# heracles-ec/heracles

Measured on AMD Instinct MI355X. Metric: map->Cl pairs/sec + mixing-matrix build sec, nside=4096 lmax=6144, higher is better.
Workload: dtype f64

## Files before the change

### heracles_amd/_lib.py

```python

from __future__ import annotations

import ctypes as C
import os
import threading

import numpy as np

_HERE = os.path.dirname(os.path.abspath(__file__))
_LIBNAME = os.environ.get("HX_LIBRARY") or os.path.join(_HERE, "libhxsht.so")
_lock = threading.Lock()
_lib = None

HX_OK = 0
HX_ERR_ARG, HX_ERR_NO_DEVICE, HX_ERR_HIP, HX_ERR_MEM, HX_ERR_UNSUPPORTED = -1, -2, -3, -4, -5

SYMBOLS = (
    "hx_version", "hx_last_error", "hx_device_count", "hx_init", "hx_set_stream",
    "hx_get_stream", "hx_set_async", "hx_synchronize", "hx_timer_start", "hx_timer_stop",
    "hx_profile_enable", "hx_profile_reset", "hx_profile_get", "hx_plan_create", "hx_set_max_lds_fft",
    "hx_plan_destroy", "hx_plan_scratch_bytes", "hx_plan_release_scratch", "hx_set_scratch_budget", "hx_plan_last_chunks", "hx_plan_mfma_flops", "hx_plan_executed_flops", "hx_executed_flops", "hx_measure_peaks", "hx_measured_mfma_clock", "hx_map2alm", "hx_map2alm_multi", "hx_map2alm_list", "hx_alm2map", "hx_copy",
    "hx_alm2cl_pairs", "hx_alm2cl_pairs_range", "hx_gauss_legendre", "hx_gauss_legendre_dd", "hx_wigner_d_table", "hx_mixmat",
    "hx_mixmat_eb", "hx_mixmat_batch", "hx_mixctx_create", "hx_mixctx_apply", "hx_mixctx_destroy", "hx_mixctx_set_bins", "hx_mixctx_apply_binned", "hx_cl2corr", "hx_corr2cl", "hx_ang2pix_ring", "hx_map_values", "hx_ud_grade", "hx_reorder", "hx_matvec", "hx_pinv", "hx_alm_resample", "hx_region_maps", "hx_alm_subtract", "hx_fits_unpack_f64", "hx_fits_pack_f64", "hx_fits_unpack_columns",
    "hx_pointsht_create", "hx_pointsht_destroy", "hx_pointsht_info", "hx_pointsht_adjoint",
    "hx_pixel_weights_size", "hx_pixel_weights_expand",
    "hx_ring_modes_size", "hx_ring_modes", "hx_legendre_from_modes", "hx_allgather_alms", "hx_host_alloc", "hx_host_free", "hx_mixmat_gemm_clock", "hx_mixmat_release", "hx_release_caches",
    "hx_cov_gram", "hx_cov_delete2", "hx_cov_shrink_sums",
    "hx_catmap_create", "hx_catmap_page", "hx_catmap_moments", "hx_catmap_finish", "hx_catmap_destroy",
    "hx_catmap_create_sel", "hx_catmap_page_sel", "hx_catmap_moments_sel", "hx_catmap_finish_sel", "hx_catmap_destroy_sel",
)


class HxError(RuntimeError):

    def __init__(self, code, msg):
        super().__init__(f"libhxsht error {code}: {msg}")
        self.code = code


def library_path() -> str:
    return _LIBNAME


def load():
# ... 5 lines not shown
            raise HxError(
                HX_ERR_NO_DEVICE,
                f"{_LIBNAME} not found: build it with `make -C heracles_amd/csrc` "
                "(hipcc, gfx950).  heracles_amd has no CPU fallback.",
            )
        try:
            import torch
        except ImportError:
            pass
        L = C.CDLL(_LIBNAME)
        vp, i, dp = C.c_void_p, C.c_int, C.c_void_p
        L.hx_version.restype = C.c_char_p
        L.hx_last_error.restype = C.c_char_p
        L.hx_get_stream.restype = vp
        L.hx_set_stream.argtypes = [vp]
        L.hx_plan_create.restype = vp
        L.hx_plan_create.argtypes = [i, i, i]
        L.hx_plan_destroy.argtypes = [vp]
        L.hx_plan_destroy.restype = None
        L.hx_plan_scratch_bytes.argtypes = [vp]
        L.hx_plan_scratch_bytes.restype = C.c_int64
        L.hx_plan_release_scratch.argtypes = [vp]
        L.hx_set_scratch_budget.argtypes = [C.c_double]
        L.hx_plan_last_chunks.argtypes = [vp]
        L.hx_plan_mfma_flops.argtypes = [vp, i, i, C.POINTER(C.c_double)]
        L.hx_plan_executed_flops.argtypes = [vp, i, i, C.POINTER(C.c_double)]
        L.hx_executed_flops.argtypes = [C.POINTER(C.c_double), i]
        L.hx_measure_peaks.argtypes = [C.POINTER(C.c_double)]
        L.hx_measured_mfma_clock.restype = C.c_double
        L.hx_map2alm.argtypes = [vp, i, i, dp, dp, dp, dp, dp, i]
        L.hx_alm2map.argtypes = [vp, i, i, dp, dp]
        L.hx_map2alm_multi.argtypes = [vp, i, vp, vp, vp, vp, dp, dp, vp]
        L.hx_map2alm_list.argtypes = [vp, i, vp, vp, vp, dp, dp, dp, dp, i]
        L.hx_copy.argtypes = [vp, vp, C.c_int64]
        L.hx_alm2cl_pairs.argtypes = [i, vp, vp, i, i, vp, vp, dp]
        L.hx_alm2cl_pairs_range.argtypes = [i, vp, vp, i, i, vp, vp, i, i, i, dp]
        L.hx_gauss_legendre.argtypes = [i, dp, dp]
        L.hx_gauss_legendre_dd.argtypes = [i, dp, dp, dp]
        L.hx_wigner_d_table.argtypes = [i, i, i, i, dp, dp]
        L.hx_mixmat.argtypes = [dp, i, i, i, i, i, i, dp]
        L.hx_mixmat_eb.argtypes = [dp, i, i, i, i, dp]
        L.hx_mixmat_batch.argtypes = [i, dp, i, i, i, i, vp, vp, vp, vp]
        L.hx_mixctx_create.restype = vp
        L.hx_mixctx_create.argtypes = [i, i, i]
        L.hx_mixctx_apply.argtypes = [vp, dp, i, i, dp]
        L.hx_mixctx_destroy.argtypes = [vp]
# ... 123 lines not shown
def release_caches():
    check(load().hx_release_caches())


def copy(dst, src):
    nb = int(src.nbytes) if hasattr(src, "nbytes") else int(src.numel() * src.element_size())
    nd = int(dst.nbytes) if hasattr(dst, "nbytes") else int(dst.numel() * dst.element_size())
    if nb != nd:
        raise ValueError(f"copy of {nb} bytes into {nd}")
    check(load().hx_copy(ptr(dst), ptr(src), nb))


def executed_flops(reset=False):
    ensure_init()
    out = (C.c_double * 2)()
    check(load().hx_executed_flops(out, 1 if reset else 0))
    return out[0], out[1]


def set_scratch_budget(nbytes: float):
    check(load().hx_set_scratch_budget(float(nbytes)))


class Timer:

    def __enter__(self):
        check(load().hx_timer_start())
        self.ms = None
        return self

    def __exit__(self, *exc):
        t = C.c_float()
        check(load().hx_timer_stop(C.byref(t)))
        self.ms = float(t.value)
        return False


def profile_enable(on=True):
    check(load().hx_profile_enable(1 if on else 0))


def profile_reset():
    check(load().hx_profile_reset())


def profile_get(name: str):
# ... 41 lines not shown
```

### heracles_amd/csrc/hx_analysis.hip

```cpp
#include <algorithm>
#include <cmath>
#include <cstdlib>
#include <cstring>

#include "hx_sht_common.h"

namespace hx {
using namespace hxfft;

constexpr int HALF_F = 1;
template <int SPIN>
struct LegCfg {
    static constexpr int NW = SPIN == 0 ? 16 : 8;
    static constexpr int NT = SPIN == 0 ? 1 : 2;
    static constexpr int NOP = SPIN == 0 ? 1 : 2;
    static constexpr int NPAR = (SPIN == 2 && HALF_F) ? 1 : 2;
};
int analysis_f_rows(int spin) { return spin == 0 ? LegCfg<0>::NPAR * LegCfg<0>::NOP : LegCfg<2>::NPAR * LegCfg<2>::NOP; }

struct LegParams {
    PlanDev P;
    const LegTask *__restrict__ tasks;
    const double *__restrict__ F;
    double *__restrict__ partial;
    int m0, ms;
    long long row0;
    int ng;
    int ncol;
    int pcol;
    const MTasks *__restrict__ of_m;
    const long long *__restrict__ arow;
    long long arow0;
    int add_all;
};

template <int SPIN>
__global__ __launch_bounds__(256) void k_fourier_combine(PlanDev P, const double2 *__restrict__ Y, int ncomp, int ng,
                                                         int ncol, int m0, int ms, const double *__restrict__ rw,
                                                         const LegTask *__restrict__ tasks, const MTasks *__restrict__ of_m,
                                                         double *__restrict__ F, int tile0)
{
    constexpr int NOP = LegCfg<SPIN>::NOP;
    __shared__ RingAtM ring_at_m[32];
    const int m = m0 + blockIdx.x * ms;
    const int ty = (int)blockIdx.y + tile0;
    const MTasks mt = of_m[m];
    if (mt.count == 0 || ty < tasks[mt.first].rb0) return;
    if (threadIdx.x < 32) ring_at_m[threadIdx.x] = ring_at_m_of(P, ty * 32 + threadIdx.x, m, rw);
    __syncthreads();
    const int rp = ty * 32 + (threadIdx.x >> 3);
    const int slot = threadIdx.x & 7;
    const bool live = rp < P.nrp;
    const RingAtM ram = ring_at_m[threadIdx.x >> 3];
    constexpr int NPAR = LegCfg<SPIN>::NPAR;
    double *row = F + (((long long)blockIdx.x * P.nrp_pad + rp) * NPAR) * NOP * ncol;
    for (int g = 0; g < ng; ++g) {
// ... 114 lines not shown
                    v[u] = make_double2(prow[j ^ 3], prow[(j + 1) ^ 3]);
                }
                if (SPIN == 2 && HALF_F && ((l + m) & 1)) {
                    if (c & 1) v[u].y = -v[u].y;
                    else v[u].x = -v[u].x;
                }
                if (alphan) al[u] = alphan[almidx(lmax, l, m)];
                if (fl) f[u] = fl[l];
            }
        }
#pragma unroll
        for (int u = 0; u < U; ++u) {
            if (!on[u]) continue;
            double2 w = v[u];
            if (alphan) { w.x *= al[u]; w.y *= al[u]; }
            if (fl) { w.x *= f[u]; w.y *= f[u]; }
            double2 *dst = alm + dsti[u];
            if (add) { const double2 o = *dst; w.x += o.x; w.y += o.y; }
            *dst = w;
        }
    }
}

template <int SPIN, int NG, int NBX, int NSUB = 1>
__global__ __launch_bounds__(256, 2) void k_legendre_duo(LegParams A, const double2 *__restrict__ coefn)
{
    using C = PipeCfg<SPIN>;
    constexpr int NW = 4, NOP = C::NOP, NCH = C::NCH, NPAIR = 16;
    constexpr int NXA = NBX > 0 ? NBX : 1;
    constexpr int DQ0 = NG * 512, DSZ = NG * 512 + NBX * 128;
    constexpr bool HALFB = SPIN == 2;
    constexpr int SB = SPIN == 2 ? DUO_SCALE_BITS2 : DUO_SCALE_BITS0;
    constexpr int GAPN = DUO_GAP >= 0 ? DUO_GAP : ((SPIN == 2 && NG == 2 && NBX == 2) ? 5 : (SPIN == 2 && NG == 2 && NBX == 1) ? 6 : (SPIN == 2 && NG == 1 && NBX == 2) ? 0 : 4);
    constexpr int GORDER = DUO_ORDER >= 0 ? DUO_ORDER : ((SPIN == 2 && NG == 2 && NBX == 2) ? 2 : (SPIN == 0 && NG == 1 && NBX == 1) ? 1 : 0);
    constexpr int NPB = HALFB ? 1 : 2;
    constexpr int TW = NSUB * DSZ > 2048 ? NSUB * DSZ : 2048;
    static_assert(NG >= 1 && NG <= 2 && TW * NW * 8 <= 81920, "two work-groups per CU");
    static_assert(SPIN == 0 || HALF_F, "spin 2: the lambda- chain carries (-1)^(l + m) lambda- (one operand row, wave-uniform coefficients)");
    __shared__ double tile[NW][TW];
    __shared__ int lead_in[2][NW];
    const PlanDev &P = A.P;
    const int m = A.m0 + blockIdx.x * A.ms, lmax = P.lmax;
    const MTasks mt = A.of_m[m];
    const int l0 = SPIN == 0 ? m : (m > 2 ? m : 2);
    const int off = (l0 + m) & 1;
    const int nblk = (lmax - l0) / LBLK + 1;
// ... 30 lines not shown
        for (int sp = 0; sp < NPAIR; ++sp) {
            const int op = SPIN == 0 ? 0 : sp & 1, q = SPIN == 0 ? sp : sp >> 1;
            const int rbq = SPIN == 0 ? 2 * w + (q >> 3) : w;
            const bool on = rbq < task.nrb;
            const long long row = (long long)blockIdx.x * P.nrp_pad + (task.rb0 + rbq) * RBLK + pipe_rho(q & 7, ak);
            if (HALFB) {
                const double *f = A.F + (row * NOP + op) * A.ncol;
#pragma unroll
                for (int g = 0; g < NG; ++g) fr[sp][0][g] = on ? f[g * NCOL + ai] : 0.0;
#pragma unroll
                for (int g = 0; g < NXA; ++g) frx[sp][0][g] = (NBX > 0 && on) ? f[NG * NCOL + 4 * g + (lane & 3)] : 0.0;
            } else {
#pragma unroll
                for (int pos = 0; pos < NPB; ++pos) {
                    const double *f = A.F + ((row * 2 + (pos ^ off)) * NOP + op) * A.ncol;
#pragma unroll
                    for (int g = 0; g < NG; ++g) fr[sp][pos][g] = on ? f[g * NCOL + ai] : 0.0;
#pragma unroll
                    for (int g = 0; g < NXA; ++g) frx[sp][pos][g] = (NBX > 0 && on) ? f[NG * NCOL + 4 * g + (lane & 3)] : 0.0;
                }
            }
        }

        double vc[NCH], vp[NCH];
        int sc[NCH];
#pragma unroll
        for (int c = 0; c < NCH; ++c) { vc[c] = 0.0; vp[c] = 0.0; sc[c] = -100; }
        if (valid) {
            if (SPIN == 0) {
                SVal a = spow(P.sth[rpl], m);
                a.v *= P.mfac[m];
                SVal b = a;
                b.v *= sqrt(2.0 * m + 3.0) * P.z[rpl];
                snorm_small(a);
                snorm_small(b);
                vc[0] = a.v; sc[0] = a.e;
                vc[NCH - 1] = b.v; sc[NCH - 1] = b.e;
            } else {
                SVal sp, sm;
                spin2_seeds(m, P.sth[rpl], P.omz[rpl], P.kfac2[m], sp, sm);
                vc[0] = (lane >> 5) ? (off ? -sm.v : sm.v) : sp.v;
                sc[0] = (lane >> 5) ? sm.e : sp.e;
            }
#pragma unroll
            for (int c = 0; c < NCH; ++c) sval_rebase<SB>(vc[c], sc[c]);
        }

        auto rec_step = [&](auto RMM, int c, int step, const double tq) __attribute__((always_inline)) {
            constexpr int RM = decltype(RMM)::value;
            if (RM != 3 && (step & 3) == 0) {
                const int hc = __double2hiint(vc[c]), hp = __double2hiint(vp[c]);
                const bool up = sc[c] < 0 && (hc & 0x7ff00000) >= 0x3ff00000;
                const int sub = up ? (SB << 20) : 0;
                const bool pz = up && (hp & 0x7ff00000) <= (SB << 20);
                vc[c] = __hiloint2double(hc - sub, __double2loint(vc[c]));
                vp[c] = pz ? 0.0 : __hiloint2double(hp - sub, __double2loint(vp[c]));
                sc[c] += up ? 1 : 0;
            }
            const double cur = (RM == 3 || sc[c] == 0) ? vc[c] : 0.0;
            const double vn = fma(tq, vc[c], -vp[c]);
            vp[c] = vc[c];
            vc[c] = vn;
            return cur;
        };
        constexpr int HB = 8;
        double *tw = &tile[w][0];
        auto recursion = [&](auto RMM, const double2 (&cl)[2]) __attribute__((always_inline)) {
            constexpr int RM = decltype(RMM)::value;
#pragma unroll
            for (int h = 0; h < LBLK / HB; ++h) {
                double cur[HB];
#pragma unroll
                for (int k = 0; k < HB; ++k) {
                    constexpr int dummy = 0; (void)dummy;
                    const int kk = HB * h + k;
                    double tq = 0.0;
                    switch (kk & 15) {
#define HX_BC(K) case K: tq = row_bcast_fmac<K>(row_bcast<K>(cl[kk >> 4].y), cl[kk >> 4].x, xx); break;
                        HX_BC(0) HX_BC(1) HX_BC(2) HX_BC(3) HX_BC(4) HX_BC(5) HX_BC(6) HX_BC(7)
                        HX_BC(8) HX_BC(9) HX_BC(10) HX_BC(11) HX_BC(12) HX_BC(13) HX_BC(14) HX_BC(15)
#undef HX_BC
                    }
                    cur[k] = rec_step(RMM, SPIN == 0 ? ((kk & 1) ? NCH - 1 : 0) : 0, SPIN == 0 ? kk >> 1 : kk, tq);
                }
                if (RM >= 2) {
#pragma unroll
                    for (int j = 0; j < HB / 2; ++j)
                        *reinterpret_cast<double2 *>(tw + pipe_tile_idx(lane, h * (HB / 2) + j)) = make_double2(cur[2 * j], cur[2 * j + 1]);
                }
                __builtin_amdgcn_sched_barrier(0);
            }
        };
        auto set_mode = [&](int b) __attribute__((always_inline)) {
            const int eb = b == 0 ? 60 : (b == 1 ? 34 : (30 - 2 * b > 8 ? 30 - 2 * b : 8));
            auto lane_dead = [&](int c) __attribute__((always_inline)) {
                if (SB == 300) return sc[c] < 0;
                const int ef = (__double2hiint(vc[c]) >> 20) & 0x7ff;
                return sc[c] <= -2 || (sc[c] == -1 && ef <= 1022 - eb);
            };
            bool dead = !valid || lane_dead(0), live = !valid || sc[0] == 0;
            if (NCH == 2) {
                dead = dead && (!valid || lane_dead(NCH - 1));
                live = live && (!valid || sc[NCH - 1] == 0);
            }
            return __all(dead) ? 1 : (__all(live) ? 3 : 2);
        };
        using I1 = std::integral_constant<int, 1>;
        using I2 = std::integral_constant<int, 2>;
        using I3 = std::integral_constant<int, 3>;

        const int fcol = tid & 15, fch = (tid >> 4) & 7, fpos = (tid >> 7) & 1;
        const int frow = (fch >> 1) + 8 * (fch & 1);
        const int qrow = tid / (4 * NXA), qcol = tid % (4 * NXA);
        double *pgrp = A.partial + (orow + 2 * frow + fpos) * A.pcol + fcol;
        double *pquad = A.partial + (orow + 2 * qrow) * A.pcol + NG * NCOL + qcol;
        double2 cnext[2] = {cfm[0], cfm[16]};
        bool started = first_group;
        int nflush = 0;
        for (int b0 = 0; b0 < nblk; b0 += NSUB) {
            double4_t acc[NSUB][NG][2];
            double accx[NSUB][NXA][2];
            bool mine = false;
#pragma unroll
            for (int sub = 0; sub < NSUB; ++sub) {
                const int b = b0 + sub;
#pragma unroll
                for (int g = 0; g < NG; ++g) acc[sub][g][0] = acc[sub][g][1] = (double4_t){0.0, 0.0, 0.0, 0.0};
#pragma unroll
                for (int g = 0; g < NXA; ++g) accx[sub][g][0] = accx[sub][g][1] = 0.0;
                if (b >= nblk) break;
                int rm = set_mode(b);
                const double2 cl[2] = {cnext[0], cnext[1]};
                if (rm == 3) recursion(I3{}, cl);
                else if (rm == 2) {
                    recursion(I2{}, cl);
                    if (SB != 300) {
                        bool lv = valid && sc[0] == 0;
                        if (NCH == 2) lv = lv || (valid && sc[NCH - 1] == 0);
                        if (!__any(lv)) rm = 1;
                    }
                } else recursion(I1{}, cl);
                cnext[0] = cfm[(b + 1) * LBLK];
                cnext[1] = cfm[(b + 1) * LBLK + 16];
                n_rec = __builtin_amdgcn_readfirstlane(n_rec + 1);
                mine = mine || rm >= 2;
                if (rm >= 2) {
                    n_mf = __builtin_amdgcn_readfirstlane(n_mf + 1);
                    if (DUO_PRIO) __builtin_amdgcn_s_setprio(0);
                    constexpr int PF = 3;
                    auto a_fetch = [&](int sp) __attribute__((always_inline)) {
                        const int op = SPIN == 0 ? 0 : sp & 1, q = SPIN == 0 ? sp : sp >> 1;
                        const int c = SPIN == 0 ? (q >> 3) * 32 + pipe_rho(q & 7, ak) : op * 32 + pipe_rho(q, ak);
                        return *reinterpret_cast<const double2 *>(tw + pipe_tile_idx(c, ai));
// ... 45 lines not shown
                                for (int g = 0; g < NG; ++g) acc[sub][g][pos] = __builtin_amdgcn_mfma_f64_16x16x4f64(a, fr[sp][HALFB ? 0 : pos][g], acc[sub][g][pos], 0, 0, 0);
#pragma unroll
                                for (int g = 0; g < NBX; ++g) accx[sub][g][pos] = __builtin_amdgcn_mfma_f64_4x4x4f64(a, frx[sp][HALFB ? 0 : pos][g], accx[sub][g][pos], 0, 0, 0);
                            }
                        }
                        __builtin_amdgcn_sched_barrier(0);
                    }
                    if (DUO_PRIO) __builtin_amdgcn_s_setprio(3);
                }
            }
            const bool two = NSUB > 1 && b0 + 1 < nblk;
            if (!started) {
                if (lane == 0) lead_in[nflush & 1][w] = mine ? 1 : 0;
                lds_barrier();
                const int4 fl = *reinterpret_cast<const int4 *>(&lead_in[nflush & 1][0]);
                ++nflush;
                started = __builtin_amdgcn_readfirstlane(fl.x | fl.y | fl.z | fl.w) != 0;
                if (!started) {
                    pgrp += (long long)NSUB * LBLK * A.pcol;
                    pquad += (long long)NSUB * LBLK * A.pcol;
                    continue;
                }
            }
#pragma unroll
            for (int sub = 0; sub < NSUB; ++sub) {
                double *dt = tw + sub * DSZ;
#pragma unroll
                for (int g = 0; g < NG; ++g)
#pragma unroll
                    for (int pos = 0; pos < 2; ++pos)
#pragma unroll
                        for (int h = 0; h < 2; ++h)
                            *reinterpret_cast<double2 *>(dt + (g * 2 + pos) * 256 + ai * 16 + (((2 * ak + h) ^ (ai & 7)) * 2)) = make_double2(acc[sub][g][pos][2 * h], acc[sub][g][pos][2 * h + 1]);
#pragma unroll
                for (int g = 0; g < NBX; ++g)
                    *reinterpret_cast<double2 *>(dt + DQ0 + ((4 * ((lane >> 2) & 3) + ak) * 4 * NBX + 4 * g + (lane & 3)) * 2) = make_double2(accx[sub][g][0], accx[sub][g][1]);
            }
            lds_barrier();
#pragma unroll
            for (int sub = 0; sub < NSUB; ++sub) {
                if (sub > 0 && !two) break;
                const long long rsub = (long long)sub * LBLK * A.pcol;
#pragma unroll
                for (int g = 0; g < NG; ++g) {
                    const double *src = &tile[0][0] + sub * DSZ + (g * 2 + fpos) * 256 + fcol * 16 + ((fch ^ (fcol & 7)) * 2);
                    double2 s4[NW];
#pragma unroll
                    for (int ww = 0; ww < NW; ++ww) s4[ww] = *reinterpret_cast<const double2 *>(src + ww * TW);
                    put(pgrp + rsub + g * NCOL, (s4[0].x + s4[1].x) + (s4[2].x + s4[3].x));
                    put(pgrp + rsub + g * NCOL + 8 * (long long)A.pcol, (s4[0].y + s4[1].y) + (s4[2].y + s4[3].y));
                }
                if (NBX > 0 && tid < 64 * NBX) {
                    double2 s4[NW];
#pragma unroll
                    for (int ww = 0; ww < NW; ++ww) s4[ww] = *reinterpret_cast<const double2 *>(&tile[0][0] + ww * TW + sub * DSZ + DQ0 + tid * 2);
                    put(pquad + rsub, (s4[0].x + s4[1].x) + (s4[2].x + s4[3].x));
                    put(pquad + rsub + A.pcol, (s4[0].y + s4[1].y) + (s4[2].y + s4[3].y));
                }
            }
            pgrp += (long long)NSUB * LBLK * A.pcol;
// ... 134 lines not shown
        ts.of_m[m].first = (int)ts.tasks.size();
        if (l0 <= lmax) {
            int first = (int)(std::lower_bound(mlim.begin(), mlim.end(), m) - mlim.begin());
            if (first >= pl->nrp) first = pl->nrp - 1;
            for (int rb = first / RBLK; rb < nrb; rb += nw) {
                LegTask t;
                t.m = m; t.rb0 = rb; t.nrb = std::min(nw, nrb - rb); t.pad = 0; t.pout = rows;
                rows += (long long)LBLK * ((lmax - l0) / LBLK + 1);
                ts.tasks.push_back(t);
            }
        }
        ts.of_m[m].count = (int)ts.tasks.size() - ts.of_m[m].first;
    }
    ts.rows_before_m[lmax + 1] = rows;
    ts.arow[lmax + 1] = arows;
    HX_TRY(upload(ts.d_tasks, ts.tasks));
    HX_TRY(upload(ts.d_of_m, ts.of_m));
    HX_TRY(upload(ts.d_arow, ts.arow));
    ts.built = true;
    return HX_OK;
}

static bool duo_shape(const SweepShape &sh) { return sh.duo != 0; }
static int sweep_pcol(const SweepShape &sh) { return sh.ncol > 2 * NCOL ? (sh.ncol + 15) / 16 * 16 : sh.ncol; }

template <int SPIN>
static int launch_duo(const SweepShape &sh, dim3 pgrid, hipStream_t st, const LegParams &A, const double2 *cn)
{
    const dim3 db(256);
    const int key = sh.ng * 10 + sh.nbx;
    if (key == 10) hipLaunchKernelGGL((k_legendre_duo<SPIN, 1, 0, 2>), pgrid, db, 0, st, A, cn);
    else if (key == 11) hipLaunchKernelGGL((k_legendre_duo<SPIN, 1, 1, 2>), pgrid, db, 0, st, A, cn);
    else if (key == 20 && SPIN == 2) hipLaunchKernelGGL((k_legendre_duo<2, 2, 0, 2>), pgrid, db, 0, st, A, cn);
    else if (key == 12 && SPIN == 2) hipLaunchKernelGGL((k_legendre_duo<2, 1, 2, 2>), pgrid, db, 0, st, A, cn);
    else if (key == 21 && SPIN == 2) hipLaunchKernelGGL((k_legendre_duo<2, 2, 1, 2>), pgrid, db, 0, st, A, cn);
    else if (key == 20) hipLaunchKernelGGL((k_legendre_duo<SPIN, 2, 0>), pgrid, db, 0, st, A, cn);
    else if (key == 22 && SPIN == 2) hipLaunchKernelGGL((k_legendre_duo<2, 2, 2>), pgrid, db, 0, st, A, cn);
    else return fail(HX_ERR_ARG, "legendre analysis: no two-group kernel for %d groups + %d blocks", sh.ng, sh.nbx);
    return HX_OK;
}

template <int SPIN>
static int launch_chunk(hx_plan *pl, hx_plan::TaskSet &ts, int m0, int m1, int nb, const SweepShape &sh, const double *d_rw,
                        const double *d_fl, int add, double2 *d_alms)
{
    const int ng = sh.ng + (sh.nbx > 0 ? 1 : 0), ncol = sh.ncol;
    const int pcol = sweep_pcol(sh);
    hipStream_t st = rt().stream;
    PlanDev P = pl->dev();
    const int t0 = ts.of_m[m0].first;
    const int t1 = ts.of_m[m1 - 1].first + ts.of_m[m1 - 1].count;
    const int ms = std::max(pl->m_step, 1), nm = (m1 - m0 + ms - 1) / ms;
    {
        ProfScope ps("fourier_combine");
        dim3 grid(nm, pl->nrp_pad / 32);
        hipLaunchKernelGGL(k_fourier_combine<SPIN>, grid, dim3(256), 0, st, P, pl->Y.as<double2>(), nb, ng, ncol, m0, ms, d_rw,
                           ts.d_tasks.as<LegTask>(), ts.d_of_m.as<MTasks>(), pl->F.as<double>(), 0);
    }
    if (t1 > t0) {
        ProfScope ps("legendre_analysis");
        ProfScope ps2(SPIN == 0 ? "legendre_analysis_s0" : "legendre_analysis_s2");
        LegParams A;
        A.P = P; A.tasks = ts.d_tasks.as<LegTask>() + t0; A.F = pl->F.as<double>(); A.partial = pl->partial.as<double>();
        A.m0 = m0; A.ms = ms; A.row0 = ts.rows_before_m[m0]; A.ng = ng; A.ncol = ncol; A.pcol = pcol;
        A.of_m = ts.d_of_m.as<MTasks>(); A.arow = ts.d_arow.as<long long>(); A.arow0 = ts.arow[m0]; A.add_all = 0;
        A.tasks = ts.d_tasks.as<LegTask>();
        const double2 *cn = SPIN == 0 ? pl->cn0.as<double2>() : pl->cn2.as<double2>();
        HX_TRY(launch_duo<SPIN>(sh, dim3((unsigned)nm), st, A, cn));
    }
    {
        ProfScope ps("alm_reduce");
        hipLaunchKernelGGL(k_alm_reduce<SPIN>, dim3(nm), dim3(256), 0, st, P, ts.d_tasks.as<LegTask>(), ts.d_of_m.as<MTasks>(),
                           pl->partial.as<double>(), ts.arow[m0], m0, ms, nb, ng, pcol, d_fl, add, d_alms, pl->nlm, ts.d_arow.as<long long>(),
                           SPIN == 0 ? pl->al0.as<double>() : pl->al2.as<double>());
    }
    HX_HIP(hipGetLastError());
    return HX_OK;
}

static bool valu_batch(int spin, int nb) { return sweep_shape(spin, nb).valu != 0; }

int valu_tasks(hx_plan *pl, int spin, hx_plan::TaskSet **out, int blocks)
{
    if (spin) HX_TRY(ensure_rec2(pl));
    if (blocks <= 0) blocks = valu_task_blocks(spin);
    if (blocks != valu_task_blocks(spin) && blocks != 8) return fail(HX_ERR_ARG, "valu_tasks: %d ring blocks per task", blocks);
    hx_plan::TaskSet &ts = blocks == 8 && blocks != valu_task_blocks(spin) ? (spin ? pl->ts[6] : pl->ts[7]) : (spin ? pl->ts[4] : pl->ts[5]);
    HX_TRY(build_task_set(pl, spin, blocks, ts));
    *out = &ts;
// ... 65 lines not shown
            ProfScope ps("alm_reduce");
            if (spin == 0)
                hipLaunchKernelGGL(k_alm_reduce<0>, dim3(nm), dim3(256), 0, rt().stream, P, ts.d_tasks.as<LegTask>(), ts.d_of_m.as<MTasks>(),
                                   pl->partial.as<double>(), ts.rows_before_m[m0], m0, ms, 1, 1, pcol, d_fl, add, d_alms + (size_t)c0 * pl->nlm, pl->nlm, nullptr, nullptr);
            else
                hipLaunchKernelGGL(k_alm_reduce<2>, dim3(nm), dim3(256), 0, rt().stream, P, ts.d_tasks.as<LegTask>(), ts.d_of_m.as<MTasks>(),
                                   pl->partial.as<double>(), ts.rows_before_m[m0], m0, ms, 2, 1, pcol, d_fl, add, d_alms + (size_t)c0 * pl->nlm, pl->nlm, nullptr, nullptr);
            HX_HIP(hipGetLastError());
        }
    return HX_OK;
}

int analysis_batch(hx_plan *pl, int spin, int nb, const double *d_maps, double2 *d_alms, const double *d_rw,
                   const double *d_pw, const double *d_fl, int add)
{
    if (valu_batch(spin, nb)) return analysis_batch_valu(pl, spin, nb, d_maps, d_alms, d_rw, d_pw, d_fl, add);
    const int sidx = spin ? 1 : 0;
    HX_TRY(build_tasks(pl, spin));
    if (spin) HX_TRY(ensure_rec2(pl));
    const SweepShape sh = sweep_shape(spin, nb);
    const bool one_set = sh.oneset || duo_shape(sh);
    if (one_set) HX_TRY(build_task_set(pl, spin, PipeCfg<2>::NW * (spin ? PipeCfg<2>::RBS : PipeCfg<0>::RBS), spin ? pl->ts[3] : pl->ts[2]));
    hx_plan::TaskSet &ts = one_set ? (spin ? pl->ts[3] : pl->ts[2]) : pl->ts[sidx];
    const int ncol = sh.ncol;
    if (pl->hsrc == nullptr && pl->nssrc == nullptr) {
        HX_TRY(pl->Y.alloc(sizeof(double2) * (size_t)pl->ny * nb));
        HX_TRY(launch_ring_subdft_maps(pl, nb, d_maps, d_pw, pl->Y.as<double2>()));
    }

    double budget = 80e9;
    if (scratch_budget_bytes() > 0.0) budget = scratch_budget_bytes();
    else {
        size_t fr = 0, tot = 0;
        if (hipMemGetInfo(&fr, &tot) == hipSuccess)
            budget = std::min(budget, 0.5 * (double)(fr + pl->F.bytes + pl->partial.bytes));
        budget = std::max(budget, 2e9);
    }
    const double f_per_m = (double)pl->nrp_pad * analysis_f_rows(spin) * ncol * sizeof(double);
    const int lmax = pl->lmax;
    const std::vector<long long> &prow = ts.arow;
    const int pcol = sweep_pcol(sh);
    std::vector<std::pair<int, int>> chunks;
    size_t maxF = 16, maxP = 16;
    const int m_end = pl->m_hi < 0 ? lmax + 1 : std::min(pl->m_hi, lmax + 1), ms = std::max(pl->m_step, 1);
    for (int m0 = std::max(pl->m_lo, 0); m0 < m_end;) {
        int last = m0;
// ... 30 lines not shown
    if (!duo_shape(sh) || sh.valu) return false;
    const double f_bytes = (double)pl->nrp_pad * analysis_f_rows(spin) * sh.ncol * sizeof(double) * (pl->lmax + 1.0);
    const double p_bytes = 0.5 * (pl->lmax + 1.0) * (pl->lmax + 2.0 + LBLK) * sweep_pcol(sh) * sizeof(double);
    double budget = 80e9;
    if (scratch_budget_bytes() > 0.0) budget = scratch_budget_bytes();
    if (f_bytes + p_bytes > budget) return false;
    size_t fr = 0, tot = 0;
    if (hipMemGetInfo(&fr, &tot) != hipSuccess) {
        (void)hipGetLastError();
        return false;
    }
    const double y_bytes = (double)pl->ny * nb * sizeof(double2), stage_bytes = 2.0 * nb * (double)pl->npix * sizeof(double);
    const double held = (double)pl->F.bytes + (double)pl->partial.bytes + (double)pl->Y.bytes + (double)pl->stage[0].bytes + (double)pl->stage[1].bytes +
                        (double)pl->stage[2].bytes;
    return f_bytes + p_bytes + y_bytes + stage_bytes <= 0.95 * ((double)fr + held);
}

int analysis_stream_plan(hx_plan *pl, int spin, int nb, int nslab, StreamSweep &s)
{
    if (!analysis_can_stream(pl, spin, nb)) return fail(HX_ERR_ARG, "analysis_stream_plan: not a streamable sweep");
    if (spin) HX_TRY(ensure_rec2(pl));
    HX_TRY(build_task_set(pl, spin, PipeCfg<2>::NW * (spin ? PipeCfg<2>::RBS : PipeCfg<0>::RBS), stream_tasks(pl, spin)));
    hx_plan::TaskSet &ts = stream_tasks(pl, spin);
    const SweepShape sh = sweep_shape(spin, nb);
    s.pl = pl; s.spin = spin; s.nb = nb;
    const int nrb = (pl->nrp + RBLK - 1) / RBLK;
    std::vector<double> cum(nrb + 1, 0.0);
    for (int rb = 0; rb < nrb; ++rb) {
        double px = 0.0;
        for (int rp = rb * RBLK; rp < std::min((rb + 1) * RBLK, pl->nrp); ++rp) px += (rp == pl->nrp - 1 ? 4.0 : 8.0) * pl->h_nsub[rp];
        cum[rb + 1] = cum[rb] + px;
    }
    nslab = std::max(1, std::min(nslab, nrb));
    s.rp_edge.assign(1, 0);
    for (int k = 1; k < nslab; ++k) {
        const int rb = (int)(std::lower_bound(cum.begin(), cum.end(), cum[nrb] * k / nslab) - cum.begin());
        if (rb * RBLK > s.rp_edge.back() && rb < nrb) s.rp_edge.push_back(rb * RBLK);
    }
    s.rp_edge.push_back(nrb * RBLK);
    s.nslab = (int)s.rp_edge.size() - 1;
    const int lmax = pl->lmax;
    std::vector<MTasks> tab((size_t)s.nslab * (lmax + 1), MTasks{0, 0});
    for (int m = 0; m <= lmax; ++m) {
        const MTasks mt = ts.of_m[m];
        int t = mt.first;
        for (int k = 0; k < s.nslab; ++k) {
// ... 26 lines not shown
{
    hx_plan *pl = s.pl;
    hx_plan::TaskSet &ts = stream_tasks(pl, SPIN);
    const SweepShape sh = sweep_shape(SPIN, s.nb);
    const int ng = sh.ng + (sh.nbx > 0 ? 1 : 0), lmax = pl->lmax, nm = lmax + 1;
    const int rp_lo = s.rp_edge[k], rp_hi = s.rp_edge[k + 1];
    hipStream_t st = rt().stream;
    PlanDev P = pl->dev();
    HX_TRY(launch_ring_subdft_maps(pl, s.nb, s.d_maps, s.d_pw, pl->Y.as<double2>(), rp_lo, std::min(rp_hi, pl->nrp)));
    {
        ProfScope ps("fourier_combine");
        const int tile_hi = k + 1 == s.nslab ? pl->nrp_pad / 32 : rp_hi / 32;
        dim3 grid(nm, tile_hi - rp_lo / 32);
        hipLaunchKernelGGL(k_fourier_combine<SPIN>, grid, dim3(256), 0, st, P, pl->Y.as<double2>(), s.nb, ng, sh.ncol, 0, 1, s.d_rw,
                           ts.d_tasks.as<LegTask>(), ts.d_of_m.as<MTasks>(), pl->F.as<double>(), rp_lo / 32);
    }
    {
        ProfScope ps("legendre_analysis");
        ProfScope ps2(SPIN == 0 ? "legendre_analysis_s0" : "legendre_analysis_s2");
        LegParams A;
        A.P = P; A.tasks = ts.d_tasks.as<LegTask>(); A.F = pl->F.as<double>(); A.partial = pl->partial.as<double>();
        A.m0 = 0; A.ms = 1; A.row0 = 0; A.ng = ng; A.ncol = sh.ncol; A.pcol = sweep_pcol(sh);
        A.of_m = s.d_of_m.as<MTasks>() + (size_t)k * (lmax + 1); A.arow = ts.d_arow.as<long long>(); A.arow0 = 0; A.add_all = 1;
        HX_TRY(launch_duo<SPIN>(sh, dim3((unsigned)nm), st, A, SPIN == 0 ? pl->cn0.as<double2>() : pl->cn2.as<double2>()));
    }
    HX_HIP(hipGetLastError());
    return HX_OK;
}

int analysis_stream_slab(StreamSweep &s, int k)
{
    if (k < 0 || k >= s.nslab) return fail(HX_ERR_ARG, "analysis_stream_slab: slab %d of %d", k, s.nslab);
    return s.spin == 0 ? stream_slab<0>(s, k) : stream_slab<2>(s, k);
}

int analysis_stream_end(StreamSweep &s)
{
    hx_plan *pl = s.pl;
    hx_plan::TaskSet &ts = stream_tasks(pl, s.spin);
    const SweepShape sh = sweep_shape(s.spin, s.nb);
    const int ng = sh.ng + (sh.nbx > 0 ? 1 : 0), nm = pl->lmax + 1, pcol = sweep_pcol(sh);
    PlanDev P = pl->dev();
    ProfScope ps("alm_reduce");
    if (s.spin == 0)
        hipLaunchKernelGGL(k_alm_reduce<0>, dim3(nm), dim3(256), 0, rt().stream, P, ts.d_tasks.as<LegTask>(), ts.d_of_m.as<MTasks>(), pl->partial.as<double>(),
                           0LL, 0, 1, s.nb, ng, pcol, s.d_fl, 0, s.d_alms, pl->nlm, ts.d_arow.as<long long>(), pl->al0.as<double>());
    else
        hipLaunchKernelGGL(k_alm_reduce<2>, dim3(nm), dim3(256), 0, rt().stream, P, ts.d_tasks.as<LegTask>(), ts.d_of_m.as<MTasks>(), pl->partial.as<double>(),
                           0LL, 0, 1, s.nb, ng, pcol, s.d_fl, 0, s.d_alms, pl->nlm, ts.d_arow.as<long long>(), pl->al2.as<double>());
    HX_HIP(hipGetLastError());
    return HX_OK;
}

}

extern "C" int hx_plan_mfma_flops(hx_plan *pl, int spin, int ncomp, double *flops)
{
    using namespace hx;
    if (!pl || !flops || ncomp < 1 || (spin != 0 && spin != 2)) return fail(HX_ERR_ARG, "hx_plan_mfma_flops: bad arguments");
    HX_TRY(ensure_ready());
    HX_TRY(build_tasks(pl, spin));
    const hx_plan::TaskSet &ts = pl->ts[spin ? 1 : 0];
    const int nop = spin ? 2 : 1, l0min = spin ? 2 : 0;
    double wave_blocks = 0.0;
    for (const LegTask &t : ts.tasks) {
        const int l0 = std::max(t.m, l0min);
        wave_blocks += (double)t.nrb * ((pl->lmax - l0) / LBLK + 1);
    }
    double per_wave_block = 0.0;
    for (int c0 = 0, nb = 0; c0 < ncomp; c0 += nb) {
        nb = analysis_next_batch(spin, ncomp - c0);
        const SweepShape sh = sweep_shape(spin, nb);
        per_wave_block += 16.0 * nop * (sh.ng * 2048.0 + sh.nbx * 512.0);
    }
    *flops = wave_blocks * per_wave_block;
    return HX_OK;
}

// ... 36 lines not shown
```

### heracles_amd/csrc/hx_sht_common.h

```cpp
#pragma once
#include <map>
#include <vector>

#include "hx_common.h"
#include "hx_fft_core.h"

namespace hx {

typedef double double4_t __attribute__((ext_vector_type(4)));

constexpr int LBLK = 32;
constexpr int NCOL = 16;
constexpr int TABLE_PAD = 512;
constexpr int NGMAX = 2;
constexpr int RBLK = 32;
constexpr double SC_BIG = 0x1p+300, SC_SMALL = 0x1p-300;

struct LegTask {
    int m;
    int rb0;
    int nrb;
    int pad;
    long long pout;
};
// ... 255 lines not shown
    int nrp = 0, nrp_pad = 0, twN = 1;
    int fft_cap = 8192;
    int last_chunks = 0;
    int eqN = 0;
    double wnorm = 0.0;
    const double2 *hsrc = nullptr;
    long long hsrc_stride = 0;
    const double4 *const *nssrc = nullptr;
    int ns_m0 = 0;
    int m_lo = 0, m_hi = -1, m_step = 1;
    long long npix = 0, ny = 0, nlm = 0;
    size_t lds_fft = 0;
    hx::DevBuf z, omz, sth, rwdef, nsub, shifted, startN, startS, bhat_off, tw, bhat, mfac, kfac2, rec0, rec2, cn0, al0, cn2, al2;
    std::vector<double> h_sth, h_z;
    std::vector<int> h_nsub;
    std::vector<long long> h_startN, h_startS;
    struct TaskSet {
        bool built = false;
        std::vector<hx::LegTask> tasks;
        std::vector<hx::MTasks> of_m;
        std::vector<long long> rows_before_m;
        std::vector<long long> arow;
        hx::DevBuf d_tasks, d_of_m, d_arow;
    } ts[8];
    struct FftClass { int M, first, count, big; };
    std::vector<FftClass> fft_classes;
    hx::DevBuf fft_rp_list;
    hx::DevBuf fft_desc;
    std::vector<int> h_fft_rp_list;
    hx::DevBuf Y, F, partial, d_dbg, resid_maps, pw_sym;
    hx::DevBuf syn_mlim0, syn_mlim2;
    hx::DevBuf syn_tab, syn_boff0, syn_boff2;
    const double *pw_checked = nullptr;
    int pw_mode = 0;
    static constexpr int NSTAGE = 3;
    hx::DevBuf stage[NSTAGE];
    hipEvent_t stage_done[NSTAGE] = {nullptr, nullptr, nullptr};
    static constexpr int NUNIT_EV = 4;
    hipEvent_t unit_up[NUNIT_EV] = {nullptr, nullptr, nullptr, nullptr};
    hx::PlanDev dev() const;
};

namespace hx {
hx_plan *plan_create_equiangular(int N, int lmax);
int ensure_rec2(hx_plan *pl);
int launch_ring_subdft_maps(hx_plan *pl, int nb, const double *d_maps, const double *d_pw, double2 *Y, int rp_lo = 0, int rp_hi = 0x7fffffff);
// ... 36 lines not shown
```

### include/hxsht.h

```cpp
#ifndef HXSHT_H
#define HXSHT_H
#include <stdint.h>
#ifdef __cplusplus
extern "C" {
#endif

#define HX_OK 0
#define HX_ERR_ARG (-1)
#define HX_ERR_NO_DEVICE (-2)
#define HX_ERR_HIP (-3)
#define HX_ERR_MEM (-4)
#define HX_ERR_UNSUPPORTED (-5)

typedef struct hx_plan hx_plan;

const char *hx_version(void);
const char *hx_last_error(void);
int hx_device_count(void);
int hx_init(int device);
int hx_set_stream(void *stream);
void *hx_get_stream(void);
int hx_set_async(int on);
int hx_synchronize(void);
int hx_copy(void *dst, const void *src, int64_t bytes);
int hx_host_alloc(int64_t bytes, void **out);
int hx_host_free(void *p);

int hx_timer_start(void);
int hx_timer_stop(float *ms);
int hx_profile_enable(int on);
int hx_profile_reset(void);
int hx_profile_get(const char *name, int *launches, double *total_ms);

hx_plan *hx_plan_create(int nside, int lmax, int max_comp);
int hx_set_max_lds_fft(int points);
void hx_plan_destroy(hx_plan *plan);
int64_t hx_plan_scratch_bytes(const hx_plan *plan);
int hx_plan_release_scratch(hx_plan *plan);
int hx_set_scratch_budget(double bytes);
int hx_plan_last_chunks(const hx_plan *plan);
int hx_measure_peaks(double *out4);
double hx_measured_mfma_clock(void);
double hx_mixmat_gemm_clock(void);
int hx_plan_mfma_flops(hx_plan *plan, int spin, int ncomp, double *flops);
int hx_plan_executed_flops(hx_plan *plan, int spin, int ncomp, double *out2);
int hx_executed_flops(double *out2, int reset);

int hx_map2alm(hx_plan *plan, int spin, int ncomp, const double *maps, double *alms,
               const double *ring_weights, const double *pix_weights, const double *fl,
               int niter);
int hx_alm2map(hx_plan *plan, int spin, int ncomp, const double *alms, double *maps);
int hx_map2alm_multi(hx_plan *plan, int njobs, const int *spins, const int *ncomps, const double *const *maps, double *const *alms,
                     const double *ring_weights, const double *pix_weights, const double *const *fls);
int hx_map2alm_list(hx_plan *plan, int nmaps, const int *spins, const double *const *maps, double *const *alms,
                    const double *ring_weights, const double *pix_weights, const double *fl0, const double *fl2, int niter);

int64_t hx_ring_modes_size(const hx_plan *plan, int count);
int hx_ring_modes(hx_plan *plan, int ncomp, const double *maps, const double *pix_weights, const double *ring_weights, int nsets,
                  const int *m_first, const int *m_count, int m_step, double *const *outs);
int hx_legendre_from_modes(hx_plan *plan, int spin, int ncomp, const double *const *comp_modes, int m_first, int m_count, int m_step,
                           double *alms, const double *fl);

// ... 107 lines not shown
```

Baseline: 422.4.

## Precompute per-task Legendre lead-in recursion state to skip dead underflow blocks

Adds a per-plan table built once by a new kernel that runs the Legendre recursion through the leading l-blocks where all lanes are still underflowed (dead mode). It stores the per-wave dead-block count and the recurrence state at that point. The main duo Legendre kernel then resumes from the stored state, zero-fills the partial output for the skipped blocks, and avoids repeating the LDS/accumulate work for idle blocks. This removes redundant lead-in recursion on every transform call, in exchange for extra device memory (capped at a fraction of free memory), a one-time build kernel, and a more complex per-wave start offset.

Result: no change. 421.3 (-0.3%).

```diff
diff --git a/heracles_amd/_lib.py b/heracles_amd/_lib.py
--- a/heracles_amd/_lib.py
+++ b/heracles_amd/_lib.py
@@ -19,7 +19,7 @@
     "hx_version", "hx_last_error", "hx_device_count", "hx_init", "hx_set_stream",
     "hx_get_stream", "hx_set_async", "hx_synchronize", "hx_timer_start", "hx_timer_stop",
     "hx_profile_enable", "hx_profile_reset", "hx_profile_get", "hx_plan_create", "hx_set_max_lds_fft",
-    "hx_plan_destroy", "hx_plan_scratch_bytes", "hx_plan_release_scratch", "hx_set_scratch_budget", "hx_plan_last_chunks", "hx_plan_mfma_flops", "hx_plan_executed_flops", "hx_executed_flops", "hx_measure_peaks", "hx_measured_mfma_clock", "hx_map2alm", "hx_map2alm_multi", "hx_map2alm_list", "hx_alm2map", "hx_copy",
+    "hx_plan_destroy", "hx_plan_scratch_bytes", "hx_plan_release_scratch", "hx_set_scratch_budget", "hx_set_leadin_table", "hx_plan_last_chunks", "hx_plan_mfma_flops", "hx_plan_executed_flops", "hx_executed_flops", "hx_measure_peaks", "hx_measured_mfma_clock", "hx_map2alm", "hx_map2alm_multi", "hx_map2alm_list", "hx_alm2map", "hx_copy",
     "hx_alm2cl_pairs", "hx_alm2cl_pairs_range", "hx_gauss_legendre", "hx_gauss_legendre_dd", "hx_wigner_d_table", "hx_mixmat",
     "hx_mixmat_eb", "hx_mixmat_batch", "hx_mixctx_create", "hx_mixctx_apply", "hx_mixctx_destroy", "hx_mixctx_set_bins", "hx_mixctx_apply_binned", "hx_cl2corr", "hx_corr2cl", "hx_ang2pix_ring", "hx_map_values", "hx_ud_grade", "hx_reorder", "hx_matvec", "hx_pinv", "hx_alm_resample", "hx_region_maps", "hx_alm_subtract", "hx_fits_unpack_f64", "hx_fits_pack_f64", "hx_fits_unpack_columns",
     "hx_pointsht_create", "hx_pointsht_destroy", "hx_pointsht_info", "hx_pointsht_adjoint",
@@ -71,6 +71,7 @@
         L.hx_plan_scratch_bytes.restype = C.c_int64
         L.hx_plan_release_scratch.argtypes = [vp]
         L.hx_set_scratch_budget.argtypes = [C.c_double]
+        L.hx_set_leadin_table.argtypes = [i]
         L.hx_plan_last_chunks.argtypes = [vp]
         L.hx_plan_mfma_flops.argtypes = [vp, i, i, C.POINTER(C.c_double)]
         L.hx_plan_executed_flops.argtypes = [vp, i, i, C.POINTER(C.c_double)]
@@ -240,6 +241,10 @@
     check(load().hx_set_scratch_budget(float(nbytes)))
 
 
+def set_leadin_table(on):
+    check(load().hx_set_leadin_table(1 if on else 0))
+
+
 class Timer:
 
     def __enter__(self):
diff --git a/heracles_amd/csrc/hx_analysis.hip b/heracles_amd/csrc/hx_analysis.hip
--- a/heracles_amd/csrc/hx_analysis.hip
+++ b/heracles_amd/csrc/hx_analysis.hip
@@ -32,6 +32,9 @@
     const long long *__restrict__ arow;
     long long arow0;
     int add_all;
+    const int *__restrict__ lead_bw;
+    const double2 *__restrict__ lead_v;
+    const int *__restrict__ lead_s;
 };
 
 template <int SPIN>
@@ -192,6 +195,119 @@
     }
 }
 
+template <int SPIN>
+struct DuoChain {
+    static constexpr int NCH = PipeCfg<SPIN>::NCH;
+    static constexpr int SB = SPIN == 2 ? DUO_SCALE_BITS2 : DUO_SCALE_BITS0;
+};
+
+template <int SPIN>
+__device__ __forceinline__ void duo_seeds(const PlanDev &P, int m, int rpl, int lane, int off, bool valid, double (&vc)[DuoChain<SPIN>::NCH],
+                                          double (&vp)[DuoChain<SPIN>::NCH], int (&sc)[DuoChain<SPIN>::NCH])
+{
+#pragma clang fp contract(off)
+    constexpr int NCH = DuoChain<SPIN>::NCH, SB = DuoChain<SPIN>::SB;
+#pragma unroll
+    for (int c = 0; c < NCH; ++c) { vc[c] = 0.0; vp[c] = 0.0; sc[c] = -100; }
+    if (valid) {
+        if (SPIN == 0) {
+            SVal a = spow(P.sth[rpl], m);
+            a.v *= P.mfac[m];
+            SVal b = a;
+            b.v *= sqrt(2.0 * m + 3.0) * P.z[rpl];
+            snorm_small(a);
+            snorm_small(b);
+            vc[0] = a.v; sc[0] = a.e;
+            vc[NCH - 1] = b.v; sc[NCH - 1] = b.e;
+        } else {
+            SVal sp, sm;
+            spin2_seeds(m, P.sth[rpl], P.omz[rpl], P.kfac2[m], sp, sm);
+            vc[0] = (lane >> 5) ? (off ? -sm.v : sm.v) : sp.v;
+            sc[0] = (lane >> 5) ? sm.e : sp.e;
+        }
+#pragma unroll
+        for (int c = 0; c < NCH; ++c) sval_rebase<SB>(vc[c], sc[c]);
+    }
+}
+
+template <int SB, int RM>
+__device__ __forceinline__ double duo_rec_step(double &vc, double &vp, int &sc, int step, const double tq)
+{
+    if (RM != 3 && (step & 3) == 0) {
+        const int hc = __double2hiint(vc), hp = __double2hiint(vp);
+        const bool up = sc < 0 && (hc & 0x7ff00000) >= 0x3ff00000;
+        const int sub = up ? (SB << 20) : 0;
+        const bool pz = up && (hp & 0x7ff00000) <= (SB << 20);
+        vc = __hiloint2double(hc - sub, __double2loint(vc));
+        vp = pz ? 0.0 : __hiloint2double(hp - sub, __double2loint(vp));
+        sc += up ? 1 : 0;
+    }
+    const double cur = (RM == 3 || sc == 0) ? vc : 0.0;
+    const double vn = fma(tq, vc, -vp);
+    vp = vc;
+    vc = vn;
+    return cur;
+}
+
+template <int SB, int NCH>
+__device__ __forceinline__ int duo_set_mode(int b, bool valid, const double (&vc)[NCH], const int (&sc)[NCH])
+{
+    const int eb = b == 0 ? 60 : (b == 1 ? 34 : (30 - 2 * b > 8 ? 30 - 2 * b : 8));
+    auto lane_dead = [&](int c) __attribute__((always_inline)) {
+        if (SB == 300) return sc[c] < 0;
+        const int ef = (__double2hiint(vc[c]) >> 20) & 0x7ff;
+        return sc[c] <= -2 || (sc[c] == -1 && ef <= 1022 - eb);
+    };
+    bool dead = !valid || lane_dead(0), live = !valid || sc[0] == 0;
+    if (NCH == 2) {
+        dead = dead && (!valid || lane_dead(NCH - 1));
+        live = live && (!valid || sc[NCH - 1] == 0);
+    }
+    return __all(dead) ? 1 : (__all(live) ? 3 : 2);
+}
+
+template <int SPIN>
+__global__ __launch_bounds__(256) void k_leadin_build(PlanDev P, const LegTask *__restrict__ tasks, int ntasks, const double2 *__restrict__ coefn,
+                                                      int *__restrict__ bw, double2 *__restrict__ tv, int *__restrict__ tsc)
+{
+    constexpr int NCH = DuoChain<SPIN>::NCH, SB = DuoChain<SPIN>::SB;
+    const int t = blockIdx.x;
+    if (t >= ntasks) return;
+    const LegTask task = tasks[t];
+    const int m = task.m, lmax = P.lmax;
+    const int l0 = SPIN == 0 ? m : (m > 2 ? m : 2);
+    const int off = (l0 + m) & 1;
+    const int nblk = (lmax - l0) / LBLK + 1;
+    const int tid = threadIdx.x, w = tid >> 6, lane = tid & 63;
+    const int rbi = SPIN == 0 ? 2 * w + (lane >> 5) : w;
+    const int rpl = (task.rb0 + rbi) * RBLK + (lane & 31);
+    const bool valid = rbi < task.nrb && rpl < P.nrp;
+    const double x = valid ? P.z[rpl] : 0.0;
+    const double xx = SPIN == 0 ? x * x : ((lane >> 5) ? -x : x);
+    double vc[NCH], vp[NCH];
+    int sc[NCH];
+    duo_seeds<SPIN>(P, m, rpl, lane, off, valid, vc, vp, sc);
+    const double2 *__restrict__ cf = coefn + almidx(lmax, 0, m) + l0 + (SPIN == 0 ? 0 : 1);
+    int b = 0;
+    for (; b < nblk; ++b) {
+        if (duo_set_mode<SB, NCH>(b, valid, vc, sc) != 1) break;
+#pragma unroll 4
+        for (int kk = 0; kk < LBLK; ++kk) {
+            const double2 pq = cf[b * LBLK + kk];
+            const double tq = fma(pq.x, xx, pq.y);
+            const int c = SPIN == 0 ? ((kk & 1) ? NCH - 1 : 0) : 0;
+            if (NCH == 2 && c) duo_rec_step<SB, 1>(vc[NCH - 1], vp[NCH - 1], sc[NCH - 1], kk >> 1, tq);
+            else duo_rec_step<SB, 1>(vc[0], vp[0], sc[0], SPIN == 0 ? kk >> 1 : kk, tq);
+        }
+    }
+    if (lane == 0) bw[4 * (long long)t + w] = b;
+#pragma unroll
+    for (int c = 0; c < NCH; ++c) {
+        tv[((long long)t * NCH + c) * 256 + tid] = make_double2(vc[c], vp[c]);
+        tsc[((long long)t * NCH + c) * 256 + tid] = sc[c];
+    }
+}
+
 template <int SPIN, int NG, int NBX, int NSUB = 1>
 __global__ __launch_bounds__(256, 2) void k_legendre_duo(LegParams A, const double2 *__restrict__ coefn)
 {
@@ -268,46 +384,28 @@
             }
         }
 
+        const int tg = mt.first + ti;
+        int bw = 0, bstart = 0;
+        if (A.lead_bw) {
+            const int4 q = *reinterpret_cast<const int4 *>(A.lead_bw + 4 * (long long)tg);
+            bw = __builtin_amdgcn_readfirstlane(w == 0 ? q.x : (w == 1 ? q.y : (w == 2 ? q.z : q.w)));
+            bstart = min(min(q.x, q.y), min(q.z, q.w));
+            bstart -= bstart % NSUB;
+        }
+
         double vc[NCH], vp[NCH];
         int sc[NCH];
-#pragma unroll
-        for (int c = 0; c < NCH; ++c) { vc[c] = 0.0; vp[c] = 0.0; sc[c] = -100; }
-        if (valid) {
-            if (SPIN == 0) {
-                SVal a = spow(P.sth[rpl], m);
-                a.v *= P.mfac[m];
-                SVal b = a;
-                b.v *= sqrt(2.0 * m + 3.0) * P.z[rpl];
-                snorm_small(a);
-                snorm_small(b);
-                vc[0] = a.v; sc[0] = a.e;
-                vc[NCH - 1] = b.v; sc[NCH - 1] = b.e;
-            } else {
-                SVal sp, sm;
-                spin2_seeds(m, P.sth[rpl], P.omz[rpl], P.kfac2[m], sp, sm);
-                vc[0] = (lane >> 5) ? (off ? -sm.v : sm.v) : sp.v;
-                sc[0] = (lane >> 5) ? sm.e : sp.e;
+        if (bw > 0) {
+#pragma unroll
+            for (int c = 0; c < NCH; ++c) {
+                const double2 s2 = A.lead_v[((long long)tg * NCH + c) * 256 + tid];
+                vc[c] = s2.x; vp[c] = s2.y;
+                sc[c] = A.lead_s[((long long)tg * NCH + c) * 256 + tid];
             }
-#pragma unroll
-            for (int c = 0; c < NCH; ++c) sval_rebase<SB>(vc[c], sc[c]);
-        }
+        } else duo_seeds<SPIN>(P, m, rpl, lane, off, valid, vc, vp, sc);
 
         auto rec_step = [&](auto RMM, int c, int step, const double tq) __attribute__((always_inline)) {
-            constexpr int RM = decltype(RMM)::value;
-            if (RM != 3 && (step & 3) == 0) {
-                const int hc = __double2hiint(vc[c]), hp = __double2hiint(vp[c]);
-                const bool up = sc[c] < 0 && (hc & 0x7ff00000) >= 0x3ff00000;
-                const int sub = up ? (SB << 20) : 0;
-                const bool pz = up && (hp & 0x7ff00000) <= (SB << 20);
-                vc[c] = __hiloint2double(hc - sub, __double2loint(vc[c]));
-                vp[c] = pz ? 0.0 : __hiloint2double(hp - sub, __double2loint(vp[c]));
-                sc[c] += up ? 1 : 0;
-            }
-            const double cur = (RM == 3 || sc[c] == 0) ? vc[c] : 0.0;
-            const double vn = fma(tq, vc[c], -vp[c]);
-            vp[c] = vc[c];
-            vc[c] = vn;
-            return cur;
+            return duo_rec_step<SB, decltype(RMM)::value>(vc[c], vp[c], sc[c], step, tq);
         };
         constexpr int HB = 8;
         double *tw = &tile[w][0];
@@ -337,20 +435,7 @@
                 __builtin_amdgcn_sched_barrier(0);
             }
         };
-        auto set_mode = [&](int b) __attribute__((always_inline)) {
-            const int eb = b == 0 ? 60 : (b == 1 ? 34 : (30 - 2 * b > 8 ? 30 - 2 * b : 8));
-            auto lane_dead = [&](int c) __attribute__((always_inline)) {
-                if (SB == 300) return sc[c] < 0;
-                const int ef = (__double2hiint(vc[c]) >> 20) & 0x7ff;
-                return sc[c] <= -2 || (sc[c] == -1 && ef <= 1022 - eb);
-            };
-            bool dead = !valid || lane_dead(0), live = !valid || sc[0] == 0;
-            if (NCH == 2) {
-                dead = dead && (!valid || lane_dead(NCH - 1));
-                live = live && (!valid || sc[NCH - 1] == 0);
-            }
-            return __all(dead) ? 1 : (__all(live) ? 3 : 2);
-        };
+        auto set_mode = [&](int b) __attribute__((always_inline)) { return duo_set_mode<SB, NCH>(b, valid, vc, sc); };
         using I1 = std::integral_constant<int, 1>;
         using I2 = std::integral_constant<int, 2>;
         using I3 = std::integral_constant<int, 3>;
@@ -360,10 +445,29 @@
         const int qrow = tid / (4 * NXA), qcol = tid % (4 * NXA);
         double *pgrp = A.partial + (orow + 2 * frow + fpos) * A.pcol + fcol;
         double *pquad = A.partial + (orow + 2 * qrow) * A.pcol + NG * NCOL + qcol;
-        double2 cnext[2] = {cfm[0], cfm[16]};
+        double2 cnext[2] = {cfm[bw * LBLK], cfm[bw * LBLK + 16]};
+        if (first_group) {
+            for (int b = 0; b < bstart; ++b) {
+#pragma unroll
+                for (int g = 0; g < NG; ++g) {
+                    pgrp[g * NCOL] = 0.0;
+                    pgrp[g * NCOL + 8 * (long long)A.pcol] = 0.0;
+                }
+                if (NBX > 0 && tid < 64 * NBX) {
+                    pquad[0] = 0.0;
+                    pquad[A.pcol] = 0.0;
+                }
+                pgrp += (long long)LBLK * A.pcol;
+                pquad += (long long)LBLK * A.pcol;
+            }
+        } else {
+            pgrp += (long long)bstart * LBLK * A.pcol;
+            pquad += (long long)bstart * LBLK * A.pcol;
+        }
         bool started = first_group;
+        bool zeroed = false;
         int nflush = 0;
-        for (int b0 = 0; b0 < nblk; b0 += NSUB) {
+        for (int b0 = bstart; b0 < nblk; b0 += NSUB) {
             double4_t acc[NSUB][NG][2];
             double accx[NSUB][NXA][2];
             bool mine = false;
@@ -375,6 +479,7 @@
 #pragma unroll
                 for (int g = 0; g < NXA; ++g) accx[sub][g][0] = accx[sub][g][1] = 0.0;
                 if (b >= nblk) break;
+                if (b < bw) continue;
                 int rm = set_mode(b);
                 const double2 cl[2] = {cnext[0], cnext[1]};
                 if (rm == 3) recursion(I3{}, cl);
@@ -466,6 +571,8 @@
                     continue;
                 }
             }
+            const bool idle = b0 + NSUB <= bw;
+            if (!(idle && zeroed))
 #pragma unroll
             for (int sub = 0; sub < NSUB; ++sub) {
                 double *dt = tw + sub * DSZ;
@@ -480,6 +587,7 @@
                 for (int g = 0; g < NBX; ++g)
                     *reinterpret_cast<double2 *>(dt + DQ0 + ((4 * ((lane >> 2) & 3) + ak) * 4 * NBX + 4 * g + (lane & 3)) * 2) = make_double2(accx[sub][g][0], accx[sub][g][1]);
             }
+            zeroed = idle;
             lds_barrier();
 #pragma unroll
             for (int sub = 0; sub < NSUB; ++sub) {
@@ -660,6 +768,42 @@
 }
 
 static bool duo_shape(const SweepShape &sh) { return sh.duo != 0; }
+
+static int g_leadin_table = 1;
+static int ensure_leadin(hx_plan *pl, int spin, hx_plan::TaskSet &ts)
+{
+    if (ts.lead_state != 0 || !g_leadin_table) return HX_OK;
+    const size_t nt = ts.tasks.size(), nch = spin ? PipeCfg<2>::NCH : PipeCfg<0>::NCH;
+    if (nt == 0) { ts.lead_state = -1; return HX_OK; }
+    const size_t bytes = nt * (4 * sizeof(int) + 256 * nch * (sizeof(double2) + sizeof(int)));
+    size_t fr = 0, tot = 0;
+    if (hipMemGetInfo(&fr, &tot) != hipSuccess) { (void)hipGetLastError(); ts.lead_state = -1; return HX_OK; }
+    if ((double)bytes > 0.125 * (double)fr || ts.lead_bw.alloc(nt * 4 * sizeof(int)) != HX_OK || ts.lead_v.alloc(nt * 256 * nch * sizeof(double2)) != HX_OK ||
+        ts.lead_s.alloc(nt * 256 * nch * sizeof(int)) != HX_OK) {
+        (void)hipGetLastError();
+        ts.lead_bw.release(); ts.lead_v.release(); ts.lead_s.release();
+        ts.lead_state = -1;
+        return HX_OK;
+    }
+    ProfScope ps("leadin_table");
+    PlanDev P = pl->dev();
+    if (spin == 0)
+        hipLaunchKernelGGL(k_leadin_build<0>, dim3((unsigned)nt), dim3(256), 0, rt().stream, P, ts.d_tasks.as<LegTask>(), (int)nt, pl->cn0.as<double2>(),
+                           ts.lead_bw.as<int>(), ts.lead_v.as<double2>(), ts.lead_s.as<int>());
+    else
+        hipLaunchKernelGGL(k_leadin_build<2>, dim3((unsigned)nt), dim3(256), 0, rt().stream, P, ts.d_tasks.as<LegTask>(), (int)nt, pl->cn2.as<double2>(),
+                           ts.lead_bw.as<int>(), ts.lead_v.as<double2>(), ts.lead_s.as<int>());
+    HX_HIP(hipGetLastError());
+    ts.lead_state = 1;
+    return HX_OK;
+}
+static void set_leadin(LegParams &A, const hx_plan::TaskSet &ts)
+{
+    const bool on = g_leadin_table && ts.lead_state == 1;
+    A.lead_bw = on ? ts.lead_bw.as<int>() : nullptr;
+    A.lead_v = on ? ts.lead_v.as<double2>() : nullptr;
+    A.lead_s = on ? ts.lead_s.as<int>() : nullptr;
+}
 static int sweep_pcol(const SweepShape &sh) { return sh.ncol > 2 * NCOL ? (sh.ncol + 15) / 16 * 16 : sh.ncol; }
 
 template <int SPIN>
@@ -703,6 +847,7 @@
         A.m0 = m0; A.ms = ms; A.row0 = ts.rows_before_m[m0]; A.ng = ng; A.ncol = ncol; A.pcol = pcol;
         A.of_m = ts.d_of_m.as<MTasks>(); A.arow = ts.d_arow.as<long long>(); A.arow0 = ts.arow[m0]; A.add_all = 0;
         A.tasks = ts.d_tasks.as<LegTask>();
+        set_leadin(A, ts);
         const double2 *cn = SPIN == 0 ? pl->cn0.as<double2>() : pl->cn2.as<double2>();
         HX_TRY(launch_duo<SPIN>(sh, dim3((unsigned)nm), st, A, cn));
     }
@@ -814,6 +959,7 @@
     const bool one_set = sh.oneset || duo_shape(sh);
     if (one_set) HX_TRY(build_task_set(pl, spin, PipeCfg<2>::NW * (spin ? PipeCfg<2>::RBS : PipeCfg<0>::RBS), spin ? pl->ts[3] : pl->ts[2]));
     hx_plan::TaskSet &ts = one_set ? (spin ? pl->ts[3] : pl->ts[2]) : pl->ts[sidx];
+    if (one_set && pl->nside >= 1) HX_TRY(ensure_leadin(pl, spin, ts));
     const int ncol = sh.ncol;
     if (pl->hsrc == nullptr && pl->nssrc == nullptr) {
         HX_TRY(pl->Y.alloc(sizeof(double2) * (size_t)pl->ny * nb));
@@ -890,6 +1036,7 @@
     if (spin) HX_TRY(ensure_rec2(pl));
     HX_TRY(build_task_set(pl, spin, PipeCfg<2>::NW * (spin ? PipeCfg<2>::RBS : PipeCfg<0>::RBS), stream_tasks(pl, spin)));
     hx_plan::TaskSet &ts = stream_tasks(pl, spin);
+    HX_TRY(ensure_leadin(pl, spin, ts));
     const SweepShape sh = sweep_shape(spin, nb);
     s.pl = pl; s.spin = spin; s.nb = nb;
     const int nrb = (pl->nrp + RBLK - 1) / RBLK;
@@ -962,6 +1109,7 @@
         A.P = P; A.tasks = ts.d_tasks.as<LegTask>(); A.F = pl->F.as<double>(); A.partial = pl->partial.as<double>();
         A.m0 = 0; A.ms = 1; A.row0 = 0; A.ng = ng; A.ncol = sh.ncol; A.pcol = sweep_pcol(sh);
         A.of_m = s.d_of_m.as<MTasks>() + (size_t)k * (lmax + 1); A.arow = ts.d_arow.as<long long>(); A.arow0 = 0; A.add_all = 1;
+        set_leadin(A, ts);
         HX_TRY(launch_duo<SPIN>(sh, dim3((unsigned)nm), st, A, SPIN == 0 ? pl->cn0.as<double2>() : pl->cn2.as<double2>()));
     }
     HX_HIP(hipGetLastError());
@@ -994,6 +1142,12 @@
 
 }
 
+extern "C" int hx_set_leadin_table(int on)
+{
+    hx::g_leadin_table = on ? 1 : 0;
+    return HX_OK;
+}
+
 extern "C" int hx_plan_mfma_flops(hx_plan *pl, int spin, int ncomp, double *flops)
 {
     using namespace hx;
diff --git a/heracles_amd/csrc/hx_sht_common.h b/heracles_amd/csrc/hx_sht_common.h
--- a/heracles_amd/csrc/hx_sht_common.h
+++ b/heracles_amd/csrc/hx_sht_common.h
@@ -301,6 +301,8 @@
         std::vector<long long> rows_before_m;
         std::vector<long long> arow;
         hx::DevBuf d_tasks, d_of_m, d_arow;
+        hx::DevBuf lead_bw, lead_v, lead_s;
+        int lead_state = 0;
     } ts[8];
     struct FftClass { int M, first, count, big; };
     std::vector<FftClass> fft_classes;
diff --git a/include/hxsht.h b/include/hxsht.h
--- a/include/hxsht.h
+++ b/include/hxsht.h
@@ -38,6 +38,7 @@
 int64_t hx_plan_scratch_bytes(const hx_plan *plan);
 int hx_plan_release_scratch(hx_plan *plan);
 int hx_set_scratch_budget(double bytes);
+int hx_set_leadin_table(int on);
 int hx_plan_last_chunks(const hx_plan *plan);
 int hx_measure_peaks(double *out4);
 double hx_measured_mfma_clock(void);
```
